# TimD1/vcfdist

Measured on AMD Instinct MI355X. Metric: supercluster-alignments/sec, higher is better.
Workload: dtype int32; 1 GPU; wgs_synth; superclusters_per_gpu=1000000, span_dist=lognormal(median 20, sigma 1.2) clip [4,10000]

## Files before the change

### vcfdist_amd/csrc/pr_api.hip

```cpp
#include <hip/hip_runtime.h>
#include <hip/hip_ext.h>
#include <dlfcn.h>

#include <algorithm>
#include <atomic>
#include <chrono>
#include <cstdarg>
#include <cstdio>
#include <cstdlib>
#include <cstring>
#include <condition_variable>
#include <deque>
#include <functional>
#include <mutex>
#include <string>
#include <thread>
#include <tuple>
#include <unordered_map>
#include <unordered_set>
#include <vector>

#include "../../include/vcfdist_pr.h"
#include "pr_device.h"
#include "pr_plan.h"
// ... 2170 lines not shown
        }
        HIPCHK(h, hipEventRecord(h->ev_slot[slot], ks));
        }
        if ((phases & 2) && !zero) {
        ls.bytes_algorithmic = ls.cells;
        rc = timed(2, ls, ks, band_bwd_name(lv), [&] {
            if (q16)
                hipLaunchKernelGGL(k_bwd_q16, dim3((cnt + 3) / 4), dim3(64), 0, ks, h->dB, h->d_descs, list, cnt,
                                   P.arena, a_i32, h->d_outs, tag, dtag, n_dev);
            else
                hipLaunchKernelGGL(band_bwd_kernel(lv), dim3(cnt), dim3(lv >= LV_C4 ? W : 64), 0,
                                   ks, h->dB, h->d_descs, list, P.arena, a_i32, h->d_outs, tag);
        });
        if (rc) return rc;
        }
        if (!(phases & 4)) return rc;
        const bool wave_walk = !q16 && (long_part || cnt < 2048);
        int64_t walk_rows_sum = 0;
        if (lv == LV_C1 && !h->seq_walk)
            for (int32_t k = 0; k < cnt && walk_rows_sum <= WSEG_MAX_ROWS; k++) walk_rows_sum += plan_desc(h, P, size_t(off) + size_t(k)).Lt;
        const bool seg_walk = lv == LV_C1 && !h->seq_walk && walk_rows_sum <= WSEG_MAX_ROWS;
        const bool row_walk = lv == LV_C1 && (wave_walk || seg_walk);
        vpr_launch_stat ws_;
        memset(&ws_, 0, sizeof(ws_));
        ws_.threads = q16 ? 16 : 64; ws_.n_units = cnt; ws_.cells_per_thread = 2;
        if (q16) {
            if (!zero) rc = timed(3, ws_, ks, "k_walk_q16", [&] {
                hipLaunchKernelGGL(k_walk_q16, dim3((cnt + 3) / 4), dim3(64), 0, ks, h->dB, h->d_descs, list, cnt,
                                   P.arena, a_i32, h->d_outs, a_path, tag, dtag, n_dev);
            });
            if (rc) return rc;
            ws_.cells_per_thread = 3;
            if (zero) {
                ws_.bytes_algorithmic = 20 * zl_rows;
                rc = timed(3, ws_, ks, "k_zero_walk", [&] {
                    hipLaunchKernelGGL(k_zero_walk, dim3((cnt + 63) / 64), dim3(64), 0, ks, h->d_descs, list, cnt, h->d_zl_hdr + zl_wave0,
                                       h->d_zl_in, h->d_zl_log, h->d_outs, a_path, (h->cfg.flags & VPR_CFG_KEEP_PATHS) ? 1 : 0, tag,
                                       h->lane_prio_rows);
                });
                if (rc) return rc;
                ws_.bytes_algorithmic = 0;
            }
            if (zero) rc = timed(3, ws_, ks, "k_zero_credit", [&] {
                hipLaunchKernelGGL(k_zero_credit, dim3((cnt + 63) / 64), dim3(64), 0, ks, h->dB, h->d_descs, list, cnt,
                                   h->d_zl_hdr + zl_wave0, h->d_zl_log, h->d_outs, h->d_secs, h->d_fp_table, h->d_jobs,
                                   h->d_njobs, h->jobs_cap, tag);
            });
            else if (cnt <= CREDIT_WAVE_MAX && !n_dev) rc = timed(3, ws_, ks, "k_credit<wave>", [&] {
                hipLaunchKernelGGL(k_credit<true>, dim3(cnt), dim3(64), 0, ks, h->dB, h->d_descs, list, cnt,
                                   h->d_outs, a_path, h->d_secs, h->d_fp_table, h->d_jobs, h->d_njobs,
                                   h->jobs_cap, dtag, tag, n_dev);
            });
            else {
                static const int head_max = [] { const char *e = exp_getenv("VPR_CREDIT_HEAD"); return e ? atoi(e) : 4096; }();
                const int32_t head = (n_dev && h->d_d1_blk && cnt > 2 * head_max) ? head_max : 0;
                if (head > 0) {
                    vpr_launch_stat wh_ = ws_;
                    wh_.n_units = head;
                    rc = timed(3, wh_, ks, "k_credit<wave>", [&] {
                        hipLaunchKernelGGL(k_credit<true>, dim3(head), dim3(64), 0, ks, h->dB, h->d_descs, list, head,
                                           h->d_outs, a_path, h->d_secs, h->d_fp_table, h->d_jobs, h->d_njobs,
                                           h->jobs_cap, dtag, tag, n_dev, 0);
                    });
                    if (rc) return rc;
                }
                rc = timed(3, ws_, ks, "k_credit<lane>", [&] {
                    hipLaunchKernelGGL(k_credit<false>, dim3((cnt - head + 63) / 64), dim3(64), 0, ks, h->dB, h->d_descs,
                                       list, cnt, h->d_outs, a_path, h->d_secs, h->d_fp_table, h->d_jobs,
                                       h->d_njobs, h->jobs_cap, dtag, tag, n_dev, int(head));
                });
            }
        } else if (row_walk) {
            static const int wseg_min_rows = [] { const char *e = exp_getenv("VPR_WSEG_MIN_ROWS"); return e ? atoi(e) : 2048; }();
            int32_t n_seg = cnt;
            if (seg_walk && long_part && wseg_min_rows > 0) {
                n_seg = 0;
                while (n_seg < cnt && plan_desc(h, P, size_t(off) + size_t(n_seg)).Lt >= wseg_min_rows) n_seg++;
            }
            if (!seg_walk || n_seg < cnt) {
                const int32_t k0 = seg_walk ? n_seg : 0;
// ... 53 lines not shown
        return rc;
    }

    void ordered_fails(const int32_t *list, int32_t nc, int32_t *out, int32_t *cnt, const int32_t *n_dev, hipStream_t ks) {
        const int nb = (nc + 255) / 256;
        hipLaunchKernelGGL(k_fails_count, dim3(nb), dim3(256), 0, ks, list, nc, h->d_outs, h->d_d1_blk, 1, n_dev);
        hipLaunchKernelGGL(k_fails_scan, dim3(1), dim3(FAILS_SCAN_NT), 0, ks, h->d_d1_blk, nb, cnt);
        hipLaunchKernelGGL(k_fails_scatter, dim3(nb), dim3(256), 0, ks, list, nc, h->d_outs, h->d_d1_blk, out, 1, n_dev);
    }

    int enqueue_d1(const int32_t *list, const int32_t *n_dev, int32_t cap, int32_t n_all, hipStream_t ks, int ph, int ztag) {
        const int nw = (cap + 63) / 64;
        vpr_launch_stat ls;
        memset(&ls, 0, sizeof(ls));
        ls.threads = 64; ls.cells_per_thread = 1; ls.n_units = cap;
        int rc = VPR_OK;
        if (ph == 1) {
            rc = timed(0, ls, ks, "k_prep_d1", [&] {
                hipLaunchKernelGGL(k_d1_hdr, dim3(nw), dim3(64), 0, ks, h->d_descs, list, n_dev, cap, h->d_outs, h->d_d1_hdr);
                hipLaunchKernelGGL(k_d1_scan, dim3(1), dim3(D1_SCAN_NT), 0, ks, h->d_d1_hdr, nw, h->d1_in_cap, h->d1_log_cap, h->d_d1_info);
                hipLaunchKernelGGL(k_prep_d1, dim3(nw), dim3(256), 0, ks, h->dB, h->d_descs, list, n_dev, cap, h->d_outs, h->d_d1_hdr, h->d_d1_in);
            });
            if (rc) return rc;
            rc = timed(1, ls, ks, "k_one_lane", [&] {
                hipLaunchKernelGGL(k_one_lane, dim3(nw), dim3(64), 0, ks, h->d_descs, list, n_dev, cap, h->d_d1_hdr, h->d_d1_in, h->d_d1_log,
                                   h->d_outs, reinterpret_cast<PathEnt *>(h->plan0.arena), (h->cfg.flags & VPR_CFG_KEEP_PATHS) ? 1 : 0, h->d_d1_info,
                                   std::max(1, h->lane_prio_rows / 4));
                hipLaunchKernelGGL(k_fwd_band_finish, dim3((cap + 255) / 256), dim3(256), 0, ks, list, cap, h->d_outs, D1_TAG, n_dev);
            });
            if (rc) return rc;
            ordered_fails(list, n_all, h->d_d1_fail, h->d_d1_info + 2, n_dev, ks);
        } else if (ph == 4) {
            ls.cells_per_thread = 3;
            rc = timed(3, ls, ks, "k_one_walk", [&] {
                hipLaunchKernelGGL(k_one_walk, dim3(nw), dim3(64), 0, ks, h->d_descs, list, n_dev, cap, h->d_d1_hdr, h->d_d1_in, h->d_d1_log,
                                   h->d_outs, reinterpret_cast<PathEnt *>(h->plan0.arena), (h->cfg.flags & VPR_CFG_KEEP_PATHS) ? 1 : 0, h->d_d1_info,
                                   std::max(1, h->lane_prio_rows / 4));
            });
            if (rc) return rc;
            rc = timed(3, ls, ks, "k_one_credit", [&] {
                hipLaunchKernelGGL(k_one_credit, dim3(nw), dim3(64), 0, ks, h->dB, h->d_descs, list, n_dev, cap, h->d_d1_hdr, h->d_d1_log,
                                   h->d_outs, h->d_secs, h->d_fp_table, h->d_jobs, h->d_njobs, h->jobs_cap, ztag);
            });
        }
        return rc;
    }

    int read_fails(int slot, int64_t fail_off, hipStream_t ls, std::vector<int32_t> &fails) {
        HIPCHK(h, x_event_sync(h, h->ev_slot[slot], SITE));
        const int32_t nf = h->hp_cnt[slot];
        if (nf > 0) {
            const size_t f0 = fails.size();
            fails.insert(fails.end(), h->hp_fail + fail_off, h->hp_fail + fail_off + nf);
            if (h->debug && nf <= (getenv("VPR_DEBUG_REJECTS") ? atoi(getenv("VPR_DEBUG_REJECTS")) : 64)) {
                for (size_t k = f0; k < fails.size(); k++) {
                    const int32_t a = fails[k];
                    AlnOut o;
                    (void)hipMemcpyAsync(&o, h->d_outs + a, sizeof(o), hipMemcpyDeviceToHost, ls);
                    (void)x_sync(h, ls, SITE);
                    const AlnDesc &d = h->descs[a];
                    fprintf(stderr, "[vpr] level %d rejected sc %d aln %d: Lq %d Lr %d Lt %d  s %d exit_min %d dq %d dr %d\n",
                            int(h->level[a]), d.sc, d.aln, d.Lq, d.Lr, d.Lt, o.s, o.exit_min, o.dist_q, o.dist_r);
                }
            }
        }
        return VPR_OK;
    }

    bool overlap(const LadderCtx &c) const { return !h->no_round_overlap && !h->no_strips && c.ls2 != nullptr && (&c - h->lad) < 2; }
    int lad_sync(LadderCtx &c) {
        HIPCHK(h, x_sync(h, c.ls, SITE));
        if (overlap(c)) HIPCHK(h, x_sync(h, c.ls2, SITE));
        return VPR_OK;
    }
    int lad_flush(LadderCtx &c, std::vector<int32_t> &out) {
// ... 899 lines not shown
```

### vcfdist_amd/csrc/pr_d1.hip

```cpp
#ifndef PR_D1_HIP_
#define PR_D1_HIP_

#define D1_TAG 9
#define D1_CLEAN ZL_CLEAN_REJECT

#define GE_ALIVE 1u
#define GE_MAT 2u
#define GE_SWP 4u
#define GE_PSLOT_SHIFT 3
#define GE_SUB 32u
#define GE_SUB_SHIFT 6
#define GE_INS 256u
#define GE_INS_SHIFT 9
#define GE_DEL 2048u
#define GE_DEL_SHIFT 12
#define GE_TP 16384u
#define GE_BWD 32768u

#define MV_SWP_R 0
#define MV_MAT 1
#define MV_SUB 2
#define MV_INS 3
#define MV_DEL 4
#define MV_SWP_Q 5
// ... 572 lines not shown
                        else { kf[p][s] = -1; kg[p][s] = -1; }
                    }
                    cg[p][0] = pgw[p][0]; cg[p][1] = pgw[p][1];
                }
                cf[0] = pf.x; cf[1] = pf.y;
            }
        };
        auto f_row = [&](int t) -> zl_u2 { return __builtin_amdgcn_raw_buffer_load_b64(rlog, (t >= 0 && t < nrow) ? logB1 + (uint32_t(t) << 9) + lane8 : ZL_OOB, 0, 0); };
        auto g_row = [&](int t) -> zl_u4 { return __builtin_amdgcn_raw_buffer_load_b128(rlog, (t >= 0 && t < nrow) ? logB2 + (uint32_t(t) << 10) + lane16 : ZL_OOB, 0, 0); };
        zl_u2 pf_n = f_row(bmax - 1);
        zl_u4 pg_n = g_row(bmax - 1);
        for (int t = bmax - 1; t >= 0; t--) {
            const bool act = t < nrow;
            const bool first = act && t == nrow - 1;
            const zl_u2 pf = pf_n;
            const zl_u4 pgv = pg_n;
            pf_n = f_row(t - 1);
            pg_n = g_row(t - 1);
            const bool upper = act && ((((cf[0] | cf[1] | pf.x | pf.y) & 0xffff0000u) | cg[0][1] | cg[1][1] | pgv.y | pgv.w) != 0u);
#ifdef D1_CLOCKS
            if (lane == 0) { atomicAdd(info + 14, 1); if (__any(upper)) atomicAdd(info + 15, 1); }
#endif
            if (__any(upper)) sc_row(S4{}, t, act, first, pf, pgv);
            else sc_row(S2{}, t, act, first, pf, pgv);
        }
        beg_plane = kf[0][0] >= 0 ? VPR_PLANE_QUERY : VPR_PLANE_REF;
        ok = ok && (kf[0][0] >= 0 || kf[1][0] >= 0);
    }

    lapck(2);
    if (ok) { AlnOut &o = outs[a]; o.beg_plane = beg_plane; o.path_len = -1; }
}

__global__ void __launch_bounds__(64, 8) k_one_walk(const AlnDesc *__restrict__ descs, const int32_t *__restrict__ list,
                                                    const int32_t *__restrict__ n_dev, int n_cap, const ZlWave *__restrict__ hdr,
                                                    const uint32_t *__restrict__ zin, uint4 *__restrict__ zlog,
                                                    AlnOut *__restrict__ outs, PathEnt *__restrict__ paths, int keep_paths,
                                                    int32_t *__restrict__ info, int prio_rows) {
    const int w = blockIdx.x, lane = threadIdx.x;
    const ZlWave H = hdr[w];
    if (H.mt <= 0) return;
    if (H.mt >= prio_rows) __builtin_amdgcn_s_setprio(2);
    const int n_list = min(*n_dev, n_cap);
    const int wi = w * 64 + lane;
    const int a_ = wi < n_list ? list[wi] : -1;
    const int a = max(a_, 0);
    const AlnDesc *dp = descs + a;
    const bool ok = a_ >= 0 && outs[a].band_ok == D1_TAG && outs[a].path_len == -1;
    const int Lq = ok ? dp->Lq : 1, Lr = ok ? dp->Lr : 1;
    const int L[2] = {Lq, Lr};
    const int nrow = ok ? dp->Lt : 0;
    int bmax = nrow;
#pragma unroll
    for (int o = 32; o; o >>= 1) bmax = max(bmax, __shfl_xor(bmax, o));
    if (bmax == 0) return;
    const auto rin = __builtin_amdgcn_make_buffer_rsrc(const_cast<uint32_t *>(zin + H.in_off), 0, 256 * (2 * H.mq + 2 * H.mr + H.mt), 0x00020000);
    const auto rlog = __builtin_amdgcn_make_buffer_rsrc(zlog + H.log_off, 0, 2560 * (H.mt + 1), 0x00020000);
    const uint32_t lane4 = uint32_t(lane) << 2, lane8 = uint32_t(lane) << 3, lane16 = uint32_t(lane) << 4;
    const uint32_t posW[2] = {0u, uint32_t(2 * H.mq) << 8};
    const uint32_t post = uint32_t(2 * H.mq + 2 * H.mr) << 8;
    const uint32_t logB1 = uint32_t(H.mt + 1) << 10;
    auto in_at = [&](uint32_t off) -> uint32_t { return __builtin_amdgcn_raw_buffer_load_b32(rin, off, 0, 0); };
    auto word_at = [&](int p, int x, bool on) -> uint32_t { return in_at(on ? posW[p] + (uint32_t(x) << 8) + lane4 : ZL_OOB); };
    auto t_at = [&](int t, bool on) -> uint32_t { return in_at(on ? post + (uint32_t(t) << 8) + lane4 : ZL_OOB); };
    const int beg_plane = ok ? outs[a].beg_plane : 0;
    auto lapck = [&](int) {};
    {
        PathEnt *path = paths + dp->path_off;
        const uint32_t logS0 = logB1;
        int hi = beg_plane, slot = 0, layer = 0, x = 0, ti = 0, mv_in = -1;
        uint32_t status = 0;
        bool wok = ok, done = !ok;
        int plen = 0;
        for (int i = 0; i <= bmax; i++) {
            const bool act = wok && !done;
            if (!__any(act)) break;
            const uint32_t mvw = __builtin_amdgcn_raw_buffer_load_b32(rlog, act ? (uint32_t(ti) << 10) + lane16 + (uint32_t(layer) << 3) + (uint32_t(hi) << 2) : ZL_OOB, 0, 0);
            const uint32_t tw = t_at(ti, act);
            const uint32_t cw = word_at(hi, x, act);
            const int trv = ZW_PTR(tw), qref = hi ? x : ZW_PTR(cw);
            uint32_t sync = 1, edit = 0;
            if (mv_in >= 0) {
                const bool diag = mv_in != MV_INS && mv_in != MV_DEL;
                const bool in_t = (tw & ZW_PV) && !(tw & ZW_PB);
                const bool in_q = hi == 0 && (cw & ZW_PV) && !(cw & ZW_PB);
                sync = (diag && !in_t && !in_q && !((tw | cw) & ZW_INS) && trv == qref) ? 1u : 0u;
                edit = (mv_in == MV_SUB || mv_in == MV_INS || mv_in == MV_DEL) ? 1u : 0u;
            }
            const uint32_t eqb = (ZW_BASE(cw) == ZW_BASE(tw) ? 1u : 0u) | ((hi || !(cw & ZW_PV)) ? 2u : 0u);
            zl_u2 st;
            st.x = uint32_t(x) | (uint32_t(hi) << 16) | (sync << 17) | (eqb << 18) | (edit << 20) | (uint32_t(i - ti) << 21);
            st.y = uint32_t(qref + 1) | (uint32_t(trv + 1) << 16);
            __builtin_amdgcn_raw_buffer_store_b64(st, rlog, act ? logS0 + (uint32_t(i) << 9) + lane8 : ZL_OOB, 0, 0);
            if ((keep_paths & 1) && act) {
                uint4 pe;
                pe.x = uint32_t(x) | (uint32_t(hi) << 31);
                pe.y = uint32_t(ti) | (sync << 31) | (edit << 30);
                pe.z = uint32_t(qref);
                pe.w = uint32_t(trv);
                *reinterpret_cast<uint4 *>(path + i) = pe;
            }
            if (act) {
                if (layer == 1 && hi == 0 && x == Lq - 1 && ti == nrow - 1) { done = true; plen = i + 1; }
                else {
                    const uint32_t m = (mvw >> (8 * slot)) & 0xffu;
                    const int rank = int(m & 7u), to = int((m >> 3) & 3u);
                    if (m == 0xffu) { status |= VPR_ST_ERR_NO_PTR; wok = false; }
                    else if (rank == MV_MAT) { x++; ti++; }
                    else if (rank == MV_SWP_R || rank == MV_SWP_Q) { x = ZW_PTR(cw) + 1; hi = 1 - hi; slot = to; ti++; }
                    else if (rank == MV_SUB) { x++; ti++; layer = 1; slot = to; }
                    else if (rank == MV_INS) { x++; layer = 1; slot = to; }
                    else { ti++; layer = 1; slot = to; }
                    mv_in = rank;
                    if (ti >= nrow || x >= L[hi]) { status |= VPR_ST_ERR_NO_PTR; wok = false; }
                }
            }
        }
        lapck(3);
        {
            const int nf = __popcll(__ballot(ok && wok && done));
            if (lane == 0 && nf) atomicAdd(info + 4, nf);
        }
        if (ok) {
            AlnOut &o = outs[a];
            wok = wok && done;
            if (!wok) status |= VPR_ST_ERR_NO_PTR;
            o.beg_plane = beg_plane;
            o.path_len = wok ? plen : 0;
            if (!wok) o.n_sec = 0;
            if (status) atomicOr(&o.status, status);
        }
    }
}

struct D1Fetch {
    const uint2 *log;
    int64_t pre_i;
    uint2 pre;
    __device__ PathEnt operator()(int64_t i) {
        const uint2 v = (i == pre_i) ? pre : log[i * 64];
        if (i > 0) { pre_i = i - 1; pre = log[(i - 1) * 64]; }
        PathEnt e;
        e.a = (v.x & 0xffffu) | (((v.x >> 16) & 1u) << 31);
        e.b = uint32_t(i - int64_t((v.x >> 21) & 1u)) | (((v.x >> 17) & 1u) << 31) | (((v.x >> 20) & 1u) << 30) | (((v.x >> 18) & 3u) << 28);
        e.qref = int(v.y & 0xffffu) - 1;
        e.tref = int(v.y >> 16) - 1;
        return e;
    }
};

__global__ void __launch_bounds__(64) k_one_credit(DevBatch B, const AlnDesc *__restrict__ descs, const int32_t *__restrict__ list,
                                                   const int32_t *__restrict__ n_dev, int n_cap, const ZlWave *__restrict__ hdr,
                                                   const uint4 *__restrict__ zlog, AlnOut *__restrict__ outs, Section *__restrict__ secs,
                                                   int32_t *const *__restrict__ fp_group, EdJob *__restrict__ jobs,
                                                   int32_t *__restrict__ n_jobs, int32_t jobs_cap, int ztag) {
    const int w = blockIdx.x, lane = threadIdx.x;
    const ZlWave H = hdr[w];
    if (H.mt <= 0) return;
    const int wi = w * 64 + lane;
    if (wi >= min(*n_dev, n_cap)) return;
    const int a = list[wi];
    if (a < 0) return;
    const AlnDesc d = descs[a];
    AlnOut &O = outs[a];
    if (d.band_pad != ztag || O.band_ok != D1_TAG) return;
    if (O.status & (VPR_ST_ERR_NO_PTR | VPR_ST_ERR_LIMIT)) return;
    D1Fetch f{reinterpret_cast<const uint2 *>(zlog + H.log_off + 64 * (int64_t(H.mt) + 1)) + lane, -1, make_uint2(0, 0)};
    credit_walk<false, D1Fetch, true>(B, d, O, a, nullptr, int64_t(O.path_len), 0u, secs, fp_group, jobs, n_jobs, jobs_cap, true, f);
}

#endif
```

### vcfdist_amd/csrc/pr_kernels.hip

```cpp
#include <hip/hip_runtime.h>
#include <stdint.h>

#include "../../include/vcfdist_pr.h"
#include "pr_device.h"
#include "pr_scan.h"

__device__ __forceinline__ bool fwd_allow(int f) { return !(f & PV) || (f & PE); }
__device__ __forceinline__ bool bwd_allow(int f) { return !(f & PV) || (f & PB); }

__global__ void __launch_bounds__(256) k_prep_scof(DevBatch B) {
    __shared__ int64_t s_off[257];
    const int which = blockIdx.y;
    const int64_t *off = which < 4 ? B.hap_off[which] : B.ref_off;
    int32_t *out = which < 4 ? B.sc_hap[which] : B.sc_ref;
    const int sc0 = blockIdx.x * 256, m = min(256, B.n_sc - sc0);
    for (int i = threadIdx.x; i <= m; i += 256) s_off[i] = off[sc0 + i];
    __syncthreads();
    const int64_t beg = s_off[0], end = s_off[m];
    for (int64_t g = beg + threadIdx.x; g < end; g += 256) {
        int lo = 0, hi = m;
        while (hi - lo > 1) {
            const int mid = (lo + hi) >> 1;
            if (s_off[mid] <= g) lo = mid; else hi = mid;
        }
// ... 639 lines not shown
            }
            return __builtin_amdgcn_readlane(rs_cur, i - rs_base);
        } else {
            return int(Rs[i]);
        }
    };
    auto ts_at = [&](int i) -> int {
        if constexpr (WAVE) {
            if (i < ts_base || i >= ts_base + 64) {
                ts_base = max(0, i - 63);
                const int x = ts_base + lane_;
                ts_cur = x < t_size ? int(Ts[x]) : 0;
            }
            return __builtin_amdgcn_readlane(ts_cur, i - ts_base);
        } else {
            return int(Ts[i]);
        }
    };

    bool clean = false;
    int64_t pl_base = -1;
    bool pl_static = false;
    auto plain_static = [&]() {
        const int qr = ccur.qref, ti = int(ccur.b & 0x0fffffffu);
        const bool have = cbase + lane_ < n;
        const bool eqb = have && qr >= 0 && qr < r_size && ti < t_size && Rs[qr] == Ts[ti];
        const int qr_up = __shfl_down(qr, 1), ti_up = __shfl_down(ti, 1);
        const bool eq_up = __shfl_down(int(eqb), 1) != 0;
        pl_static = have && lane_ < 63 && cbase + lane_ + 1 < n && (ccur.b >> 31) && !((ccur.b >> 30) & 1u) &&
                    qr_up == qr + 1 && ti_up == ti + 1 && eq_up;
        pl_base = cbase;
    };
    while (sync_idx >= 0) {
        if constexpr (WAVE && !EXT) {
            if (clean && sync_idx < n) {
                if (pl_base != cbase) plain_static();
                const int l = int(sync_idx - cbase);
                const bool plain = pl_static && ccur.qref >= query_var_pos && ccur.tref >= truth_var_pos;
                const unsigned long long below = (l == 63) ? ~0ull : ((2ull << l) - 1ull);
                const unsigned long long stop = ~__ballot(plain) & below;
                const int run = stop ? l - (63 - __builtin_clzll(stop)) : l + 1;
                if (run > 0) {
                    const int lj = l - run + 1;
                    prev_qref = __builtin_amdgcn_readlane(ccur.qref, lj);
                    prev_tref = __builtin_amdgcn_readlane(ccur.tref, lj);
                    cur_b = uint32_t(__builtin_amdgcn_readlane(int(ccur.b), lj));
                    prev_hi = int(uint32_t(__builtin_amdgcn_readlane(int(ccur.a), lj)) >> 31);
                    prev_ti = int(cur_b & 0x0fffffffu);
                    prev_sync_ref_idx = prev_qref + 1;
                    prev_sync_truth_idx = prev_ti + 1;
                    eq_cur = (cur_b >> 28) & 3u;
                    sync_idx -= run;
                    if (sync_idx < 0) break;
                    cur_hi = prev_hi;
                    const PathEnt e = fetch(sync_idx);
                    cur_b = e.b;
                    eq_next = eq_cur; eq_cur = (e.b >> 28) & 3u;
                    nx_qref = prev_qref; nx_ti = prev_ti;
                    prev_qri = int(e.a & 0x7fffffffu);
                    prev_hi = int(e.a >> 31);
                    prev_ti = int(e.b & 0x0fffffffu);
                    prev_qref = e.qref;
                    prev_tref = e.tref;
                    continue;
                }
            }
// ... 710 lines not shown
```

### vcfdist_amd/csrc/pr_zl.hip

```cpp
#ifndef PR_ZL_HIP_
#define PR_ZL_HIP_
#include <type_traits>


#define ZW_PTR(w) (int((w) & 0xffffu) - 1)
#define ZW_BASE(w) (((w) >> 16) & 0x7fu)
#define ZW_PV (1u << 23)
#define ZW_PB (1u << 24)
#define ZW_PE (1u << 25)
#define ZW_INS (1u << 26)
#define ZW_TP (1u << 27)
__device__ __forceinline__ bool zw_fwd_allow(uint32_t w) { return !(w & ZW_PV) || (w & ZW_PE); }
__device__ __forceinline__ bool zw_bwd_allow(uint32_t w) { return !(w & ZW_PV) || (w & ZW_PB); }

#define ZE_ALIVE 1u
#define ZE_HASMAT 2u
#define ZE_HASSWP 4u
#define ZE_PSLOT_SHIFT 3
#define ZE_TP 32u
#define ZE_BWD 64u

#define ZL_MAXLEN 65000
#define ZL_CLEAN_REJECT (-1)

// ... 304 lines not shown
    auto row_at = [&](int r) -> zl_u2 { return log_row(r, r >= 0 && r < nrow); };
    zl_u2 lastpre = row_at(bmax - 1);
    zl_u2 rA = row_at(bmax - 2), rB = row_at(bmax - 3), rC = row_at(bmax - 4), rD = zl_u2{0, 0};
    auto bwd_step = [&](int t, const zl_u2 &pre_reg, zl_u2 &next_reg) {
        const bool act = t >= 1 && t < nrow;
        const bool first = t == nrow - 1 && t >= 1;
        if (first) {
            const int ep = endq >= 0 ? 0 : 1, es = endq >= 0 ? endq : endr;
            cur = lastpre;
#pragma unroll
            for (int p = 0; p < 2; p++) {
#pragma unroll
                for (int s = 0; s < 4; s++) sc[p][s] = (p == ep && s == es) ? 0 : -1;
            }
        }
        next_reg = row_at(t - 4);
        const zl_u2 pre = pre_reg;
        const bool upper = act && (((cur.x | cur.y | pre.x | pre.y) & 0xffff0000u) != 0u);
        if (__any(upper)) bwd_row(std::integral_constant<int, 4>{}, t, act, pre);
        else bwd_row(std::integral_constant<int, 2>{}, t, act, pre);
        lastpre = pre;
    };
    for (int t = bmax - 1; t >= 1; t -= 4) {
        bwd_step(t, rA, rD);
        bwd_step(t - 1, rB, rA);
        bwd_step(t - 2, rC, rB);
        bwd_step(t - 3, rD, rC);
    }
    const int beg_plane = sc[0][0] >= 0 ? VPR_PLANE_QUERY : VPR_PLANE_REF;

    if (ok) outs[a].beg_plane = beg_plane;
}

__global__ void __launch_bounds__(64, 8) k_zero_walk(const AlnDesc *__restrict__ descs, const int32_t *__restrict__ list, int n_list,
                                                  const ZlWave *__restrict__ hdr, const uint32_t *__restrict__ zin,
                                                  uint4 *__restrict__ zlog, AlnOut *__restrict__ outs, PathEnt *__restrict__ paths,
                                                  int keep_paths, int tag, int prio_rows) {
    const int w = blockIdx.x, lane = threadIdx.x;
    const ZlWave H = hdr[w];
    if (H.mt >= prio_rows) __builtin_amdgcn_s_setprio(2);
    const int wi = w * 64 + lane;
    const int a_ = wi < n_list ? list[wi] : -1;
    const bool live = a_ >= 0;
    const int a = max(a_, 0);
    const AlnDesc *dp = descs + a;
    const auto rin = __builtin_amdgcn_make_buffer_rsrc(const_cast<uint32_t *>(zin + H.in_off), 0, 256 * (H.mq + H.mr + H.mt), 0x00020000);
    const auto rlog = __builtin_amdgcn_make_buffer_rsrc(zlog + H.log_off, 0, 1280 * H.mt, 0x00020000);
    const uint32_t lane4 = uint32_t(lane) << 2, lane8 = uint32_t(lane) << 3;
    const uint32_t pos0[2] = {0u, uint32_t(H.mq) << 8}, post = uint32_t(H.mq + H.mr) << 8;
    const uint32_t logP0 = uint32_t(H.mt) << 9, logS0 = logP0 + (uint32_t(H.mt) << 8);
    auto in_at = [&](uint32_t off) -> uint32_t { return __builtin_amdgcn_raw_buffer_load_b32(rin, off, 0, 0); };
    const bool ok = live && dp->band_pad == tag && outs[a].band_ok == tag;
    const int nrow = ok ? dp->Lt : 0;
    int bmax = nrow;
#pragma unroll
    for (int o = 32; o; o >>= 1) bmax = max(bmax, __shfl_xor(bmax, o));
    if (bmax == 0) return;
    const int beg_plane = ok ? outs[a].beg_plane : 0;
    PathEnt *path = paths + dp->path_off;
    int hi = beg_plane, slot = 0, mv_in = 0, x = 0;
    uint32_t status = 0;
    bool wok = ok;
    for (int t = 0; t < bmax; t++) {
        const bool act = wok && t < nrow;
        const uint32_t ppw = __builtin_amdgcn_raw_buffer_load_b32(rlog, (act && t + 1 < nrow) ? logP0 + (uint32_t(t) << 8) + lane4 : ZL_OOB, 0, 0);
        const uint32_t tw = in_at(act ? post + (uint32_t(t) << 8) + lane4 : ZL_OOB);
        const uint32_t cw = in_at(act ? pos0[hi] + (uint32_t(x) << 8) + lane4 : ZL_OOB);
        const int trv = ZW_PTR(tw), qref = hi ? x : ZW_PTR(cw);
        uint32_t sync = 1;
        if (mv_in) {
            const bool in_t = (tw & ZW_PV) && !(tw & ZW_PB);
            const bool in_q = hi == 0 && (cw & ZW_PV) && !(cw & ZW_PB);
            sync = (!in_t && !in_q && !((tw | cw) & ZW_INS) && trv == qref) ? 1u : 0u;
        }
        const uint32_t eqb = (ZW_BASE(cw) == ZW_BASE(tw) ? 1u : 0u) | ((hi || !(cw & ZW_PV)) ? 2u : 0u);
        zl_u2 st;
        st.x = uint32_t(x) | (uint32_t(hi) << 16) | (sync << 17) | (eqb << 18);
        st.y = uint32_t(qref + 1) | (uint32_t(trv + 1) << 16);
        __builtin_amdgcn_raw_buffer_store_b64(st, rlog, act ? logS0 + (uint32_t(t) << 9) + lane8 : ZL_OOB, 0, 0);
        if ((keep_paths & 1) && act) {
            uint4 pe;
            pe.x = uint32_t(x) | (uint32_t(hi) << 31);
            pe.y = uint32_t(t) | (sync << 31);
            pe.z = uint32_t(qref);
            pe.w = uint32_t(trv);
            *reinterpret_cast<uint4 *>(path + t) = pe;
        }
        if (act && t + 1 < nrow) {
            const uint32_t nb = (ppw >> (4 * ((hi << 2) | slot))) & 15u;
            if (hi == 1 && (nb & 2u)) { hi = 0; slot = int(nb >> 2); x = ZW_PTR(cw) + 1; }
            else if (nb & 1u) { x = x + 1; }
            else if (hi == 0 && (nb & 2u)) { hi = 1; slot = int(nb >> 2); x = ZW_PTR(cw) + 1; }
            else { status |= VPR_ST_ERR_NO_PTR; wok = false; }
            mv_in = 1;
        }
    }
    if (ok) {
        AlnOut &o = outs[a];
        o.path_len = wok ? nrow : 0;
        if (!wok) o.n_sec = 0;
        if (status) atomicOr(&o.status, status);
    }
}

struct ZlFetch {
    const uint2 *log;
    int64_t pre_i;
    uint2 pre;
    __device__ PathEnt operator()(int64_t i) {
        const uint2 v = (i == pre_i) ? pre : log[i * 64];
        if (i > 0) { pre_i = i - 1; pre = log[(i - 1) * 64]; }
        PathEnt e;
        e.a = (v.x & 0xffffu) | (((v.x >> 16) & 1u) << 31);
        e.b = uint32_t(i) | (((v.x >> 17) & 1u) << 31) | (((v.x >> 18) & 3u) << 28);
        e.qref = int(v.y & 0xffffu) - 1;
        e.tref = int(v.y >> 16) - 1;
        return e;
    }
};

__global__ void __launch_bounds__(64) k_zero_credit(DevBatch B, const AlnDesc *__restrict__ descs, const int32_t *__restrict__ list,
                                                    int n_list, const ZlWave *__restrict__ hdr, const uint4 *__restrict__ zlog,
                                                    AlnOut *__restrict__ outs, Section *__restrict__ secs,
                                                    int32_t *const *__restrict__ fp_group, EdJob *__restrict__ jobs,
                                                    int32_t *__restrict__ n_jobs, int32_t jobs_cap, int tag) {
    const int w = blockIdx.x, lane = threadIdx.x;
    const int wi = w * 64 + lane;
    if (wi >= n_list) return;
    const int a = list[wi];
    if (a < 0) return;
    const AlnDesc d = descs[a];
    AlnOut &O = outs[a];
    if (d.band_pad != tag || O.band_ok != tag) return;
    if (O.status & (VPR_ST_ERR_NO_PTR | VPR_ST_ERR_LIMIT)) return;
    const ZlWave H = hdr[w];
    ZlFetch f{reinterpret_cast<const uint2 *>(zlog + H.log_off + 48 * int64_t(H.mt)) + lane, -1, make_uint2(0, 0)};
    credit_walk<false, ZlFetch, true>(B, d, O, a, nullptr, int64_t(O.path_len), 0u, secs, fp_group, jobs, n_jobs, jobs_cap, true, f);
}

#endif
```

Measured before the change: 194.1 million supercluster-alignments/s.

## Fuse walk and credit kernels with run-length path log and prefetched walk loads

Merges the zero-lane and one-lane traceback walk kernels with their credit kernels, so each lane runs credit_walk right after its walk, reading its own freshly written log. The per-row path log becomes run-length encoded: consecutive matching diagonal steps collapse into one record, read back through a RunFetch that can also skip plain runs. The walk loop is unrolled by four with a rotating set of prefetched loads, reissuing loads when the position jumps. This removes a launch and most log traffic per batch, at the cost of higher register pressure and more complex, divergent fused kernels.

```diff
diff --git a/vcfdist_amd/csrc/pr_api.hip b/vcfdist_amd/csrc/pr_api.hip
--- a/vcfdist_amd/csrc/pr_api.hip
+++ b/vcfdist_amd/csrc/pr_api.hip
@@ -2226,20 +2226,14 @@
             if (rc) return rc;
             ws_.cells_per_thread = 3;
             if (zero) {
-                ws_.bytes_algorithmic = 20 * zl_rows;
-                rc = timed(3, ws_, ks, "k_zero_walk", [&] {
-                    hipLaunchKernelGGL(k_zero_walk, dim3((cnt + 63) / 64), dim3(64), 0, ks, h->d_descs, list, cnt, h->d_zl_hdr + zl_wave0,
-                                       h->d_zl_in, h->d_zl_log, h->d_outs, a_path, (h->cfg.flags & VPR_CFG_KEEP_PATHS) ? 1 : 0, tag,
+                ws_.bytes_algorithmic = 12 * zl_rows;
+                rc = timed(3, ws_, ks, "k_zero_walk_credit", [&] {
+                    hipLaunchKernelGGL(k_zero_walk_credit, dim3((cnt + 63) / 64), dim3(64), 0, ks, h->dB, h->d_descs, list, cnt,
+                                       h->d_zl_hdr + zl_wave0, h->d_zl_in, h->d_zl_log, h->d_outs, a_path, h->d_secs, h->d_fp_table,
+                                       h->d_jobs, h->d_njobs, h->jobs_cap, (h->cfg.flags & VPR_CFG_KEEP_PATHS) ? 1 : 0, tag,
                                        h->lane_prio_rows);
                 });
-                if (rc) return rc;
-                ws_.bytes_algorithmic = 0;
-            }
-            if (zero) rc = timed(3, ws_, ks, "k_zero_credit", [&] {
-                hipLaunchKernelGGL(k_zero_credit, dim3((cnt + 63) / 64), dim3(64), 0, ks, h->dB, h->d_descs, list, cnt,
-                                   h->d_zl_hdr + zl_wave0, h->d_zl_log, h->d_outs, h->d_secs, h->d_fp_table, h->d_jobs,
-                                   h->d_njobs, h->jobs_cap, tag);
-            });
+            }
             else if (cnt <= CREDIT_WAVE_MAX && !n_dev) rc = timed(3, ws_, ks, "k_credit<wave>", [&] {
                 hipLaunchKernelGGL(k_credit<true>, dim3(cnt), dim3(64), 0, ks, h->dB, h->d_descs, list, cnt,
                                    h->d_outs, a_path, h->d_secs, h->d_fp_table, h->d_jobs, h->d_njobs,
@@ -2359,15 +2353,11 @@
             ordered_fails(list, n_all, h->d_d1_fail, h->d_d1_info + 2, n_dev, ks);
         } else if (ph == 4) {
             ls.cells_per_thread = 3;
-            rc = timed(3, ls, ks, "k_one_walk", [&] {
-                hipLaunchKernelGGL(k_one_walk, dim3(nw), dim3(64), 0, ks, h->d_descs, list, n_dev, cap, h->d_d1_hdr, h->d_d1_in, h->d_d1_log,
-                                   h->d_outs, reinterpret_cast<PathEnt *>(h->plan0.arena), (h->cfg.flags & VPR_CFG_KEEP_PATHS) ? 1 : 0, h->d_d1_info,
+            rc = timed(3, ls, ks, "k_one_walk_credit", [&] {
+                hipLaunchKernelGGL(k_one_walk_credit, dim3(nw), dim3(64), 0, ks, h->dB, h->d_descs, list, n_dev, cap, h->d_d1_hdr, h->d_d1_in,
+                                   h->d_d1_log, h->d_outs, reinterpret_cast<PathEnt *>(h->plan0.arena), h->d_secs, h->d_fp_table, h->d_jobs,
+                                   h->d_njobs, h->jobs_cap, (h->cfg.flags & VPR_CFG_KEEP_PATHS) ? 1 : 0, h->d_d1_info, ztag,
                                    std::max(1, h->lane_prio_rows / 4));
-            });
-            if (rc) return rc;
-            rc = timed(3, ls, ks, "k_one_credit", [&] {
-                hipLaunchKernelGGL(k_one_credit, dim3(nw), dim3(64), 0, ks, h->dB, h->d_descs, list, n_dev, cap, h->d_d1_hdr, h->d_d1_log,
-                                   h->d_outs, h->d_secs, h->d_fp_table, h->d_jobs, h->d_njobs, h->jobs_cap, ztag);
             });
         }
         return rc;
diff --git a/vcfdist_amd/csrc/pr_d1.hip b/vcfdist_amd/csrc/pr_d1.hip
--- a/vcfdist_amd/csrc/pr_d1.hip
+++ b/vcfdist_amd/csrc/pr_d1.hip
@@ -628,11 +628,15 @@
     if (ok) { AlnOut &o = outs[a]; o.beg_plane = beg_plane; o.path_len = -1; }
 }
 
-__global__ void __launch_bounds__(64, 8) k_one_walk(const AlnDesc *__restrict__ descs, const int32_t *__restrict__ list,
-                                                    const int32_t *__restrict__ n_dev, int n_cap, const ZlWave *__restrict__ hdr,
-                                                    const uint32_t *__restrict__ zin, uint4 *__restrict__ zlog,
-                                                    AlnOut *__restrict__ outs, PathEnt *__restrict__ paths, int keep_paths,
-                                                    int32_t *__restrict__ info, int prio_rows) {
+struct D1Slot { uint32_t m, t, c; };
+
+__global__ void __launch_bounds__(64, 8) k_one_walk_credit(DevBatch B, const AlnDesc *__restrict__ descs, const int32_t *__restrict__ list,
+                                                        const int32_t *__restrict__ n_dev, int n_cap, const ZlWave *__restrict__ hdr,
+                                                        const uint32_t *__restrict__ zin, uint4 *__restrict__ zlog,
+                                                        AlnOut *__restrict__ outs, PathEnt *__restrict__ paths, Section *__restrict__ secs,
+                                                        int32_t *const *__restrict__ fp_group, EdJob *__restrict__ jobs,
+                                                        int32_t *__restrict__ n_jobs, int32_t jobs_cap, int keep_paths,
+                                                        int32_t *__restrict__ info, int ztag, int prio_rows) {
     const int w = blockIdx.x, lane = threadIdx.x;
     const ZlWave H = hdr[w];
     if (H.mt <= 0) return;
@@ -644,7 +648,6 @@
     const AlnDesc *dp = descs + a;
     const bool ok = a_ >= 0 && outs[a].band_ok == D1_TAG && outs[a].path_len == -1;
     const int Lq = ok ? dp->Lq : 1, Lr = ok ? dp->Lr : 1;
-    const int L[2] = {Lq, Lr};
     const int nrow = ok ? dp->Lt : 0;
     int bmax = nrow;
 #pragma unroll
@@ -653,116 +656,116 @@
     const auto rin = __builtin_amdgcn_make_buffer_rsrc(const_cast<uint32_t *>(zin + H.in_off), 0, 256 * (2 * H.mq + 2 * H.mr + H.mt), 0x00020000);
     const auto rlog = __builtin_amdgcn_make_buffer_rsrc(zlog + H.log_off, 0, 2560 * (H.mt + 1), 0x00020000);
     const uint32_t lane4 = uint32_t(lane) << 2, lane8 = uint32_t(lane) << 3, lane16 = uint32_t(lane) << 4;
-    const uint32_t posW[2] = {0u, uint32_t(2 * H.mq) << 8};
+    const uint32_t posR = uint32_t(2 * H.mq) << 8;
     const uint32_t post = uint32_t(2 * H.mq + 2 * H.mr) << 8;
     const uint32_t logB1 = uint32_t(H.mt + 1) << 10;
     auto in_at = [&](uint32_t off) -> uint32_t { return __builtin_amdgcn_raw_buffer_load_b32(rin, off, 0, 0); };
-    auto word_at = [&](int p, int x, bool on) -> uint32_t { return in_at(on ? posW[p] + (uint32_t(x) << 8) + lane4 : ZL_OOB); };
-    auto t_at = [&](int t, bool on) -> uint32_t { return in_at(on ? post + (uint32_t(t) << 8) + lane4 : ZL_OOB); };
     const int beg_plane = ok ? outs[a].beg_plane : 0;
-    auto lapck = [&](int) {};
+    PathEnt *path = paths + dp->path_off;
+    const uint32_t logS0 = logB1;
+    int hi = beg_plane, slot = 0, layer = 0, x = 0, ti = 0, mv_in = -1;
+    uint32_t status = 0;
+    bool wok = ok, done = !ok;
+    int plen = 0;
+    zl_u2 run = zl_u2{0, 0}, rprev = zl_u2{0, 0};
+    uint32_t rc = 0;
+    int32_t nrec = 0;
+    auto request = [&](D1Slot &s, int rt, int px) {
+        const bool on = wok && !done && rt < nrow;
+        s.m = __builtin_amdgcn_raw_buffer_load_b32(rlog, on ? (uint32_t(rt) << 10) + lane16 + (uint32_t(layer) << 3) + (uint32_t(hi) << 2) : ZL_OOB, 0, 0);
+        s.t = in_at(on ? post + (uint32_t(rt) << 8) + lane4 : ZL_OOB);
+        s.c = in_at(on ? (hi ? posR : 0u) + (uint32_t(px) << 8) + lane4 : ZL_OOB);
+    };
+    D1Slot sA, sB, sC, sD;
+    request(sA, 0, 0); request(sB, 1, 1); request(sC, 2, 2); request(sD, 3, 3);
+    auto wstep = [&](int i, D1Slot &S, D1Slot &S1, D1Slot &S2, D1Slot &S3) -> bool {
+        const bool act = wok && !done && i <= bmax;
+        if (!__any(act)) return false;
+        const uint32_t mvw = S.m, tw = S.t, cw = S.c;
+        const int trv = ZW_PTR(tw), qref = hi ? x : ZW_PTR(cw);
+        uint32_t sync = 1, edit = 0;
+        if (mv_in >= 0) {
+            const bool diag = mv_in != MV_INS && mv_in != MV_DEL;
+            const bool in_t = (tw & ZW_PV) && !(tw & ZW_PB);
+            const bool in_q = hi == 0 && (cw & ZW_PV) && !(cw & ZW_PB);
+            sync = (diag && !in_t && !in_q && !((tw | cw) & ZW_INS) && trv == qref) ? 1u : 0u;
+            edit = (mv_in == MV_SUB || mv_in == MV_INS || mv_in == MV_DEL) ? 1u : 0u;
+        }
+        const uint32_t eqb = (ZW_BASE(cw) == ZW_BASE(tw) ? 1u : 0u) | ((hi || !(cw & ZW_PV)) ? 2u : 0u);
+        zl_u2 st;
+        st.x = uint32_t(x) | (uint32_t(hi) << 16) | (sync << 17) | (eqb << 18) | (edit << 20) | ((uint32_t(i - ti) & 1u) << 21);
+        st.y = uint32_t(qref + 1) | (uint32_t(trv + 1) << 16);
+        const uint32_t n1 = rc + 1u;
+        const bool follows = sync && !edit && eqb == 3u && rc < RUN_MAX && ((st.x ^ run.x) & ((1u << 16) | (1u << 21))) == 0u &&
+                             uint32_t(x) == (run.x & 0xffffu) + n1 && uint32_t(qref + 1) == (run.y & 0xffffu) + n1 &&
+                             uint32_t(trv + 1) == (run.y >> 16) + n1;
+        const bool put = act && i > 0 && !follows;
+        const zl_u2 rec = zl_u2{run.x | (rc << RUN_SHIFT), run.y};
+        __builtin_amdgcn_raw_buffer_store_b64(rec, rlog, put ? logS0 + (uint32_t(nrec) << 9) + lane8 : ZL_OOB, 0, 0);
+        if (put) { rprev = rec; nrec++; }
+        if (act) {
+            if (i > 0 && follows) rc = n1;
+            else { run = st; rc = 0; }
+        }
+        if ((keep_paths & 1) && act) {
+            uint4 pe;
+            pe.x = uint32_t(x) | (uint32_t(hi) << 31);
+            pe.y = uint32_t(ti) | (sync << 31) | (edit << 30);
+            pe.z = uint32_t(qref);
+            pe.w = uint32_t(trv);
+            *reinterpret_cast<uint4 *>(path + i) = pe;
+        }
+        bool off_diag = false;
+        if (act) {
+            if (layer == 1 && hi == 0 && x == Lq - 1 && ti == nrow - 1) { done = true; plen = i + 1; }
+            else {
+                const uint32_t m = (mvw >> (8 * slot)) & 0xffu;
+                const int rank = int(m & 7u), to = int((m >> 3) & 3u);
+                if (m == 0xffu) { status |= VPR_ST_ERR_NO_PTR; wok = false; }
+                else if (rank == MV_MAT) { x++; ti++; }
+                else if (rank == MV_SWP_R || rank == MV_SWP_Q) { x = ZW_PTR(cw) + 1; hi = 1 - hi; slot = to; ti++; }
+                else if (rank == MV_SUB) { x++; ti++; layer = 1; slot = to; }
+                else if (rank == MV_INS) { x++; layer = 1; slot = to; }
+                else { ti++; layer = 1; slot = to; }
+                mv_in = rank;
+                if (ti >= nrow || x >= (hi ? Lr : Lq)) { status |= VPR_ST_ERR_NO_PTR; wok = false; }
+                off_diag = wok && rank != MV_MAT;
+            }
+        }
+        request(S, ti + 3, x + 3);
+        if (off_diag) {
+            request(S1, ti, x);
+            request(S2, ti + 1, x + 1);
+            request(S3, ti + 2, x + 2);
+        }
+        return true;
+    };
+    for (int i = 0; i <= bmax; i += 4) {
+        if (!wstep(i, sA, sB, sC, sD)) break;
+        if (!wstep(i + 1, sB, sC, sD, sA)) break;
+        if (!wstep(i + 2, sC, sD, sA, sB)) break;
+        if (!wstep(i + 3, sD, sA, sB, sC)) break;
+    }
     {
-        PathEnt *path = paths + dp->path_off;
-        const uint32_t logS0 = logB1;
-        int hi = beg_plane, slot = 0, layer = 0, x = 0, ti = 0, mv_in = -1;
-        uint32_t status = 0;
-        bool wok = ok, done = !ok;
-        int plen = 0;
-        for (int i = 0; i <= bmax; i++) {
-            const bool act = wok && !done;
-            if (!__any(act)) break;
-            const uint32_t mvw = __builtin_amdgcn_raw_buffer_load_b32(rlog, act ? (uint32_t(ti) << 10) + lane16 + (uint32_t(layer) << 3) + (uint32_t(hi) << 2) : ZL_OOB, 0, 0);
-            const uint32_t tw = t_at(ti, act);
-            const uint32_t cw = word_at(hi, x, act);
-            const int trv = ZW_PTR(tw), qref = hi ? x : ZW_PTR(cw);
-            uint32_t sync = 1, edit = 0;
-            if (mv_in >= 0) {
-                const bool diag = mv_in != MV_INS && mv_in != MV_DEL;
-                const bool in_t = (tw & ZW_PV) && !(tw & ZW_PB);
-                const bool in_q = hi == 0 && (cw & ZW_PV) && !(cw & ZW_PB);
-                sync = (diag && !in_t && !in_q && !((tw | cw) & ZW_INS) && trv == qref) ? 1u : 0u;
-                edit = (mv_in == MV_SUB || mv_in == MV_INS || mv_in == MV_DEL) ? 1u : 0u;
-            }
-            const uint32_t eqb = (ZW_BASE(cw) == ZW_BASE(tw) ? 1u : 0u) | ((hi || !(cw & ZW_PV)) ? 2u : 0u);
-            zl_u2 st;
-            st.x = uint32_t(x) | (uint32_t(hi) << 16) | (sync << 17) | (eqb << 18) | (edit << 20) | (uint32_t(i - ti) << 21);
-            st.y = uint32_t(qref + 1) | (uint32_t(trv + 1) << 16);
-            __builtin_amdgcn_raw_buffer_store_b64(st, rlog, act ? logS0 + (uint32_t(i) << 9) + lane8 : ZL_OOB, 0, 0);
-            if ((keep_paths & 1) && act) {
-                uint4 pe;
-                pe.x = uint32_t(x) | (uint32_t(hi) << 31);
-                pe.y = uint32_t(ti) | (sync << 31) | (edit << 30);
-                pe.z = uint32_t(qref);
-                pe.w = uint32_t(trv);
-                *reinterpret_cast<uint4 *>(path + i) = pe;
-            }
-            if (act) {
-                if (layer == 1 && hi == 0 && x == Lq - 1 && ti == nrow - 1) { done = true; plen = i + 1; }
-                else {
-                    const uint32_t m = (mvw >> (8 * slot)) & 0xffu;
-                    const int rank = int(m & 7u), to = int((m >> 3) & 3u);
-                    if (m == 0xffu) { status |= VPR_ST_ERR_NO_PTR; wok = false; }
-                    else if (rank == MV_MAT) { x++; ti++; }
-                    else if (rank == MV_SWP_R || rank == MV_SWP_Q) { x = ZW_PTR(cw) + 1; hi = 1 - hi; slot = to; ti++; }
-                    else if (rank == MV_SUB) { x++; ti++; layer = 1; slot = to; }
-                    else if (rank == MV_INS) { x++; layer = 1; slot = to; }
-                    else { ti++; layer = 1; slot = to; }
-                    mv_in = rank;
-                    if (ti >= nrow || x >= L[hi]) { status |= VPR_ST_ERR_NO_PTR; wok = false; }
-                }
-            }
-        }
-        lapck(3);
-        {
-            const int nf = __popcll(__ballot(ok && wok && done));
-            if (lane == 0 && nf) atomicAdd(info + 4, nf);
-        }
-        if (ok) {
-            AlnOut &o = outs[a];
-            wok = wok && done;
-            if (!wok) status |= VPR_ST_ERR_NO_PTR;
-            o.beg_plane = beg_plane;
-            o.path_len = wok ? plen : 0;
-            if (!wok) o.n_sec = 0;
-            if (status) atomicOr(&o.status, status);
-        }
-    }
+        const int nf = __popcll(__ballot(ok && wok && done));
+        if (lane == 0 && nf) atomicAdd(info + 4, nf);
+    }
+    wok = wok && done;
+    if (ok) {
+        AlnOut &o = outs[a];
+        if (!wok) status |= VPR_ST_ERR_NO_PTR;
+        o.beg_plane = beg_plane;
+        o.path_len = wok ? plen : 0;
+        if (!wok) o.n_sec = 0;
+        if (status) atomicOr(&o.status, status);
+    }
+    if (!ok || !wok) return;
+    const AlnDesc d = descs[a];
+    if (d.band_pad != ztag) return;
+    AlnOut &O = outs[a];
+    if (O.status & (VPR_ST_ERR_NO_PTR | VPR_ST_ERR_LIMIT)) return;
+    RunFetch f{rlog, logS0 + lane8, nrec, int64_t(plen) - 1 - int64_t(rc), zl_u2{run.x | (rc << RUN_SHIFT), run.y}, rprev};
+    credit_walk<false, RunFetch, true>(B, d, O, a, nullptr, int64_t(plen), 0u, secs, fp_group, jobs, n_jobs, jobs_cap, true, f);
 }
 
-struct D1Fetch {
-    const uint2 *log;
-    int64_t pre_i;
-    uint2 pre;
-    __device__ PathEnt operator()(int64_t i) {
-        const uint2 v = (i == pre_i) ? pre : log[i * 64];
-        if (i > 0) { pre_i = i - 1; pre = log[(i - 1) * 64]; }
-        PathEnt e;
-        e.a = (v.x & 0xffffu) | (((v.x >> 16) & 1u) << 31);
-        e.b = uint32_t(i - int64_t((v.x >> 21) & 1u)) | (((v.x >> 17) & 1u) << 31) | (((v.x >> 20) & 1u) << 30) | (((v.x >> 18) & 3u) << 28);
-        e.qref = int(v.y & 0xffffu) - 1;
-        e.tref = int(v.y >> 16) - 1;
-        return e;
-    }
-};
-
-__global__ void __launch_bounds__(64) k_one_credit(DevBatch B, const AlnDesc *__restrict__ descs, const int32_t *__restrict__ list,
-                                                   const int32_t *__restrict__ n_dev, int n_cap, const ZlWave *__restrict__ hdr,
-                                                   const uint4 *__restrict__ zlog, AlnOut *__restrict__ outs, Section *__restrict__ secs,
-                                                   int32_t *const *__restrict__ fp_group, EdJob *__restrict__ jobs,
-                                                   int32_t *__restrict__ n_jobs, int32_t jobs_cap, int ztag) {
-    const int w = blockIdx.x, lane = threadIdx.x;
-    const ZlWave H = hdr[w];
-    if (H.mt <= 0) return;
-    const int wi = w * 64 + lane;
-    if (wi >= min(*n_dev, n_cap)) return;
-    const int a = list[wi];
-    if (a < 0) return;
-    const AlnDesc d = descs[a];
-    AlnOut &O = outs[a];
-    if (d.band_pad != ztag || O.band_ok != D1_TAG) return;
-    if (O.status & (VPR_ST_ERR_NO_PTR | VPR_ST_ERR_LIMIT)) return;
-    D1Fetch f{reinterpret_cast<const uint2 *>(zlog + H.log_off + 64 * (int64_t(H.mt) + 1)) + lane, -1, make_uint2(0, 0)};
-    credit_walk<false, D1Fetch, true>(B, d, O, a, nullptr, int64_t(O.path_len), 0u, secs, fp_group, jobs, n_jobs, jobs_cap, true, f);
-}
-
 #endif
diff --git a/vcfdist_amd/csrc/pr_kernels.hip b/vcfdist_amd/csrc/pr_kernels.hip
--- a/vcfdist_amd/csrc/pr_kernels.hip
+++ b/vcfdist_amd/csrc/pr_kernels.hip
@@ -695,6 +695,35 @@
         pl_base = cbase;
     };
     while (sync_idx >= 0) {
+        if constexpr (!WAVE && EXT) {
+            if (clean && sync_idx < n) {
+                const int64_t lo = xf.plain_lo(sync_idx, query_var_pos, truth_var_pos, r_size);
+                if (lo <= sync_idx) {
+                    const PathEnt e0 = xf.entry(lo);
+                    prev_qref = e0.qref;
+                    prev_tref = e0.tref;
+                    cur_b = e0.b;
+                    prev_hi = int(e0.a >> 31);
+                    prev_ti = int(cur_b & 0x0fffffffu);
+                    prev_sync_ref_idx = prev_qref + 1;
+                    prev_sync_truth_idx = prev_ti + 1;
+                    eq_cur = (cur_b >> 28) & 3u;
+                    sync_idx = lo - 1;
+                    if (sync_idx < 0) break;
+                    cur_hi = prev_hi;
+                    const PathEnt e = fetch(sync_idx);
+                    cur_b = e.b;
+                    eq_next = eq_cur; eq_cur = (e.b >> 28) & 3u;
+                    nx_qref = prev_qref; nx_ti = prev_ti;
+                    prev_qri = int(e.a & 0x7fffffffu);
+                    prev_hi = int(e.a >> 31);
+                    prev_ti = int(e.b & 0x0fffffffu);
+                    prev_qref = e.qref;
+                    prev_tref = e.tref;
+                    continue;
+                }
+            }
+        }
         if constexpr (WAVE && !EXT) {
             if (clean && sync_idx < n) {
                 if (pl_base != cbase) plain_static();
diff --git a/vcfdist_amd/csrc/pr_zl.hip b/vcfdist_amd/csrc/pr_zl.hip
--- a/vcfdist_amd/csrc/pr_zl.hip
+++ b/vcfdist_amd/csrc/pr_zl.hip
@@ -360,10 +360,51 @@
     if (ok) outs[a].beg_plane = beg_plane;
 }
 
-__global__ void __launch_bounds__(64, 8) k_zero_walk(const AlnDesc *__restrict__ descs, const int32_t *__restrict__ list, int n_list,
-                                                  const ZlWave *__restrict__ hdr, const uint32_t *__restrict__ zin,
-                                                  uint4 *__restrict__ zlog, AlnOut *__restrict__ outs, PathEnt *__restrict__ paths,
-                                                  int keep_paths, int tag, int prio_rows) {
+#define RUN_SHIFT 22
+#define RUN_MAX 1023u
+
+struct RunFetch {
+    __amdgpu_buffer_rsrc_t log;
+    uint32_t col;
+    int32_t k;
+    int64_t h;
+    zl_u2 cur, pre;
+    __device__ void seek(int64_t i) {
+        while (i < h) {
+            k--;
+            cur = pre;
+            pre = __builtin_amdgcn_raw_buffer_load_b64(log, k >= 1 ? col + (uint32_t(k - 1) << 9) : ZL_OOB, 0, 0);
+            h -= 1 + int64_t(cur.x >> RUN_SHIFT);
+        }
+    }
+    __device__ PathEnt entry(int64_t i) const {
+        const uint32_t j = uint32_t(i - h), hx = cur.x;
+        const uint32_t flags = j ? ((1u << 31) | (3u << 28)) : ((((hx >> 17) & 1u) << 31) | (((hx >> 20) & 1u) << 30) | (((hx >> 18) & 3u) << 28));
+        PathEnt e;
+        e.a = ((hx & 0xffffu) + j) | (((hx >> 16) & 1u) << 31);
+        e.b = uint32_t(i - int64_t((hx >> 21) & 1u)) | flags;
+        e.qref = int(cur.y & 0xffffu) - 1 + int(j);
+        e.tref = int(cur.y >> 16) - 1 + int(j);
+        return e;
+    }
+    __device__ PathEnt operator()(int64_t i) { seek(i); return entry(i); }
+    __device__ int64_t plain_lo(int64_t i, int qvp, int tvp, int r_size) const {
+        const int c = int(cur.x >> RUN_SHIFT);
+        const int qh = int(cur.y & 0xffffu) - 1, th = int(cur.y >> 16) - 1;
+        const int head = (((cur.x >> 17) & 1u) && !((cur.x >> 20) & 1u)) ? 0 : 1;
+        const int64_t top = h + min(c - 1, r_size - 2 - qh);
+        return i <= top ? h + max(max(head, qvp - qh), tvp - th) : i + 1;
+    }
+};
+
+struct ZwSlot { uint32_t p, t, c; };
+
+__global__ void __launch_bounds__(64, 8) k_zero_walk_credit(DevBatch B, const AlnDesc *__restrict__ descs, const int32_t *__restrict__ list,
+                                                         int n_list, const ZlWave *__restrict__ hdr, const uint32_t *__restrict__ zin,
+                                                         uint4 *__restrict__ zlog, AlnOut *__restrict__ outs, PathEnt *__restrict__ paths,
+                                                         Section *__restrict__ secs, int32_t *const *__restrict__ fp_group,
+                                                         EdJob *__restrict__ jobs, int32_t *__restrict__ n_jobs, int32_t jobs_cap,
+                                                         int keep_paths, int tag, int prio_rows) {
     const int w = blockIdx.x, lane = threadIdx.x;
     const ZlWave H = hdr[w];
     if (H.mt >= prio_rows) __builtin_amdgcn_s_setprio(2);
@@ -375,7 +416,7 @@
     const auto rin = __builtin_amdgcn_make_buffer_rsrc(const_cast<uint32_t *>(zin + H.in_off), 0, 256 * (H.mq + H.mr + H.mt), 0x00020000);
     const auto rlog = __builtin_amdgcn_make_buffer_rsrc(zlog + H.log_off, 0, 1280 * H.mt, 0x00020000);
     const uint32_t lane4 = uint32_t(lane) << 2, lane8 = uint32_t(lane) << 3;
-    const uint32_t pos0[2] = {0u, uint32_t(H.mq) << 8}, post = uint32_t(H.mq + H.mr) << 8;
+    const uint32_t posR = uint32_t(H.mq) << 8, post = uint32_t(H.mq + H.mr) << 8;
     const uint32_t logP0 = uint32_t(H.mt) << 9, logS0 = logP0 + (uint32_t(H.mt) << 8);
     auto in_at = [&](uint32_t off) -> uint32_t { return __builtin_amdgcn_raw_buffer_load_b32(rin, off, 0, 0); };
     const bool ok = live && dp->band_pad == tag && outs[a].band_ok == tag;
@@ -389,11 +430,20 @@
     int hi = beg_plane, slot = 0, mv_in = 0, x = 0;
     uint32_t status = 0;
     bool wok = ok;
-    for (int t = 0; t < bmax; t++) {
+    zl_u2 run = zl_u2{0, 0}, rprev = zl_u2{0, 0};
+    uint32_t rc = 0;
+    int32_t nrec = 0;
+    auto request = [&](ZwSlot &s, int r, int px) {
+        const bool on = wok && r < nrow;
+        s.p = __builtin_amdgcn_raw_buffer_load_b32(rlog, (on && r + 1 < nrow) ? logP0 + (uint32_t(r) << 8) + lane4 : ZL_OOB, 0, 0);
+        s.t = in_at(on ? post + (uint32_t(r) << 8) + lane4 : ZL_OOB);
+        s.c = in_at(on ? (hi ? posR : 0u) + (uint32_t(px) << 8) + lane4 : ZL_OOB);
+    };
+    ZwSlot sA, sB, sC, sD;
+    request(sA, 0, 0); request(sB, 1, 1); request(sC, 2, 2); request(sD, 3, 3);
+    auto wstep = [&](int t, ZwSlot &S, ZwSlot &S1, ZwSlot &S2, ZwSlot &S3) {
         const bool act = wok && t < nrow;
-        const uint32_t ppw = __builtin_amdgcn_raw_buffer_load_b32(rlog, (act && t + 1 < nrow) ? logP0 + (uint32_t(t) << 8) + lane4 : ZL_OOB, 0, 0);
-        const uint32_t tw = in_at(act ? post + (uint32_t(t) << 8) + lane4 : ZL_OOB);
-        const uint32_t cw = in_at(act ? pos0[hi] + (uint32_t(x) << 8) + lane4 : ZL_OOB);
+        const uint32_t ppw = S.p, tw = S.t, cw = S.c;
         const int trv = ZW_PTR(tw), qref = hi ? x : ZW_PTR(cw);
         uint32_t sync = 1;
         if (mv_in) {
@@ -405,7 +455,17 @@
         zl_u2 st;
         st.x = uint32_t(x) | (uint32_t(hi) << 16) | (sync << 17) | (eqb << 18);
         st.y = uint32_t(qref + 1) | (uint32_t(trv + 1) << 16);
-        __builtin_amdgcn_raw_buffer_store_b64(st, rlog, act ? logS0 + (uint32_t(t) << 9) + lane8 : ZL_OOB, 0, 0);
+        const uint32_t n1 = rc + 1u;
+        const bool follows = sync && eqb == 3u && rc < RUN_MAX && ((st.x ^ run.x) & (1u << 16)) == 0u && uint32_t(x) == (run.x & 0xffffu) + n1 &&
+                             uint32_t(qref + 1) == (run.y & 0xffffu) + n1 && uint32_t(trv + 1) == (run.y >> 16) + n1;
+        const bool put = act && t > 0 && !follows;
+        const zl_u2 rec = zl_u2{run.x | (rc << RUN_SHIFT), run.y};
+        __builtin_amdgcn_raw_buffer_store_b64(rec, rlog, put ? logS0 + (uint32_t(nrec) << 9) + lane8 : ZL_OOB, 0, 0);
+        if (put) { rprev = rec; nrec++; }
+        if (act) {
+            if (t > 0 && follows) rc = n1;
+            else { run = st; rc = 0; }
+        }
         if ((keep_paths & 1) && act) {
             uint4 pe;
             pe.x = uint32_t(x) | (uint32_t(hi) << 31);
@@ -414,14 +474,27 @@
             pe.w = uint32_t(trv);
             *reinterpret_cast<uint4 *>(path + t) = pe;
         }
+        bool swp = false;
         if (act && t + 1 < nrow) {
             const uint32_t nb = (ppw >> (4 * ((hi << 2) | slot))) & 15u;
-            if (hi == 1 && (nb & 2u)) { hi = 0; slot = int(nb >> 2); x = ZW_PTR(cw) + 1; }
+            if (hi == 1 && (nb & 2u)) { hi = 0; slot = int(nb >> 2); x = ZW_PTR(cw) + 1; swp = true; }
             else if (nb & 1u) { x = x + 1; }
-            else if (hi == 0 && (nb & 2u)) { hi = 1; slot = int(nb >> 2); x = ZW_PTR(cw) + 1; }
+            else if (hi == 0 && (nb & 2u)) { hi = 1; slot = int(nb >> 2); x = ZW_PTR(cw) + 1; swp = true; }
             else { status |= VPR_ST_ERR_NO_PTR; wok = false; }
             mv_in = 1;
         }
+        request(S, t + 4, x + 3);
+        if (swp) {
+            S1.c = in_at((hi ? posR : 0u) + (uint32_t(x) << 8) + lane4);
+            S2.c = in_at((hi ? posR : 0u) + (uint32_t(x + 1) << 8) + lane4);
+            S3.c = in_at((hi ? posR : 0u) + (uint32_t(x + 2) << 8) + lane4);
+        }
+    };
+    for (int t = 0; t < bmax; t += 4) {
+        wstep(t, sA, sB, sC, sD);
+        wstep(t + 1, sB, sC, sD, sA);
+        wstep(t + 2, sC, sD, sA, sB);
+        wstep(t + 3, sD, sA, sB, sC);
     }
     if (ok) {
         AlnOut &o = outs[a];
@@ -429,41 +502,12 @@
         if (!wok) o.n_sec = 0;
         if (status) atomicOr(&o.status, status);
     }
+    if (!ok || !wok) return;
+    AlnOut &O = outs[a];
+    if (O.status & (VPR_ST_ERR_NO_PTR | VPR_ST_ERR_LIMIT)) return;
+    const AlnDesc d = descs[a];
+    RunFetch f{rlog, logS0 + lane8, nrec, int64_t(nrow) - 1 - int64_t(rc), zl_u2{run.x | (rc << RUN_SHIFT), run.y}, rprev};
+    credit_walk<false, RunFetch, true>(B, d, O, a, nullptr, int64_t(nrow), 0u, secs, fp_group, jobs, n_jobs, jobs_cap, true, f);
 }
 
-struct ZlFetch {
-    const uint2 *log;
-    int64_t pre_i;
-    uint2 pre;
-    __device__ PathEnt operator()(int64_t i) {
-        const uint2 v = (i == pre_i) ? pre : log[i * 64];
-        if (i > 0) { pre_i = i - 1; pre = log[(i - 1) * 64]; }
-        PathEnt e;
-        e.a = (v.x & 0xffffu) | (((v.x >> 16) & 1u) << 31);
-        e.b = uint32_t(i) | (((v.x >> 17) & 1u) << 31) | (((v.x >> 18) & 3u) << 28);
-        e.qref = int(v.y & 0xffffu) - 1;
-        e.tref = int(v.y >> 16) - 1;
-        return e;
-    }
-};
-
-__global__ void __launch_bounds__(64) k_zero_credit(DevBatch B, const AlnDesc *__restrict__ descs, const int32_t *__restrict__ list,
-                                                    int n_list, const ZlWave *__restrict__ hdr, const uint4 *__restrict__ zlog,
-                                                    AlnOut *__restrict__ outs, Section *__restrict__ secs,
-                                                    int32_t *const *__restrict__ fp_group, EdJob *__restrict__ jobs,
-                                                    int32_t *__restrict__ n_jobs, int32_t jobs_cap, int tag) {
-    const int w = blockIdx.x, lane = threadIdx.x;
-    const int wi = w * 64 + lane;
-    if (wi >= n_list) return;
-    const int a = list[wi];
-    if (a < 0) return;
-    const AlnDesc d = descs[a];
-    AlnOut &O = outs[a];
-    if (d.band_pad != tag || O.band_ok != tag) return;
-    if (O.status & (VPR_ST_ERR_NO_PTR | VPR_ST_ERR_LIMIT)) return;
-    const ZlWave H = hdr[w];
-    ZlFetch f{reinterpret_cast<const uint2 *>(zlog + H.log_off + 48 * int64_t(H.mt)) + lane, -1, make_uint2(0, 0)};
-    credit_walk<false, ZlFetch, true>(B, d, O, a, nullptr, int64_t(O.path_len), 0u, secs, fp_group, jobs, n_jobs, jobs_cap, true, f);
-}
-
 #endif
```

New measurement: 203.0 million supercluster-alignments/s (median of 6 runs). 1.05x the previous value.
